# OATML-Markslab/ProteinGym

Hardware: AMD Instinct MI355X
Metric: mutants scored/sec (ESM-1v 650M masked-marginal) (higher is better)
Workload: dtype f16x3 (fp32 operands split into 2 fp16 planes, 3 fp16 MFMAs per product, fp32 accumulate)

## Files before the change

proteingym_amd/csrc/api_model.hip:

```cpp
#include "model.h"

namespace pgmi {

static thread_local char g_err[1024] = "";
void set_error(const char* fmt, ...) {
    va_list ap;
    va_start(ap, fmt);
    vsnprintf(g_err, sizeof(g_err), fmt, ap);
    va_end(ap);
}

int prof_drain(pgmi_model* m) {
    if (m->events_used == 0) return PGMI_OK;
    PGMI_HIP(hipStreamSynchronize(m->stream));
    for (size_t i = 0; i < m->events_used; ++i) {
        float ms = 0.f;
        PGMI_HIP(hipEventElapsedTime(&ms, m->events[i].start, m->events[i].stop));
        m->prof_ms[m->events[i].cls] += ms;
    }
    m->events_used = 0;
    return PGMI_OK;
}

int check_cfg(const pgmi_config* c) {
// ... 312 lines not shown
                         : cfg->arch == PGMI_ARCH_ESM3 ? esm3_weight_count(cfg, arch_arg)
                         : cfg->arch == PGMI_ARCH_ESMIF1 ? if1_weight_count(cfg, arch_arg) : pgmi_weight_count(cfg);
    if (need < 0) { set_error("causal decoder pos_kind %d: must be PGMI_GPT_POS_ROTARY or PGMI_GPT_POS_LEARNED", arch_arg); return PGMI_EINVAL; }
    if (!w || n_weights != need) {
        set_error("weight blob has %lld elements, config needs %lld", (long long)n_weights, (long long)need);
        return PGMI_EINVAL;
    }
    const int ndev = pgmi_device_count();
    if (ndev <= 0) { set_error("no HIP device visible (libpgmi has no CPU fallback)"); return PGMI_ENODEV; }
    if (device < 0 || device >= ndev) { set_error("device %d out of range (%d visible)", device, ndev); return PGMI_EINVAL; }
    PGMI_HIP(hipSetDevice(device));
    pgmi_model* m = new pgmi_model();
    m->cfg = *cfg;
    m->device = device;
    if (hipStreamCreateWithFlags(&m->stream, hipStreamNonBlocking) != hipSuccess) { set_error("hipStreamCreate failed"); delete m; return PGMI_EHIP; }
    m->dh = cfg->embed_dim / cfg->heads;
    m->rot_halves = m->dh > 2 * kHeadDim ? 4 : m->dh > kHeadDim ? 2 : 1;
    m->Hs = cfg->heads * m->rot_halves;
    m->Da = m->Hs * kHeadDim;
    m->ln_eps = cfg->ln_eps > 0.f ? cfg->ln_eps : 1e-5f;
    m->max_rows = std::max(cfg->max_rows > 0 ? cfg->max_rows : 98304, 2048);
    const size_t V = cfg->vocab;
    const std::vector<float> zeros(std::max({3 * (size_t)m->Da, (V + 63) / 64 * 64, (size_t)cfg->embed_dim, V, (size_t)cfg->heads}), 0.0f);
    rc = dev_upload(m->allocs, &m->zeros, zeros.data(), zeros.size());
    m->fc1_cols = cfg->ffn_dim;
    if (!rc) switch (cfg->arch) {
        case PGMI_ARCH_TRANCEPTION: rc = create_tranception(m, cfg, w, n_weights); break;
        case PGMI_ARCH_MSA: rc = create_msa(m, cfg, w, n_weights); break;
        case PGMI_ARCH_PROGEN2: rc = create_progen2(m, cfg, w, n_weights, arch_arg); break;
        case PGMI_ARCH_GPT: rc = create_gpt(m, cfg, w, n_weights, arch_arg); break;
        case PGMI_ARCH_ESMC: rc = create_esmc(m, cfg, w, n_weights); break;
        case PGMI_ARCH_SAPROT: rc = create_saprot(m, cfg, w, n_weights, arch_arg); break;
        case PGMI_ARCH_POET: rc = create_poet(m, cfg, w, n_weights, arch_arg); break;
        case PGMI_ARCH_PROGEN3: rc = create_progen3(m, cfg, w, n_weights, pg3); break;
        case PGMI_ARCH_ESM3: rc = create_esm3(m, cfg, w, n_weights, arch_arg); break;
        case PGMI_ARCH_ESMIF1: rc = create_esmif1(m, cfg, w, n_weights, arch_arg); break;
        default: rc = create_esm(m, cfg, w, n_weights);
    }
    if (!rc) rc = alloc_workspace(m);
    if (rc) { pgmi_model_destroy(m); return rc; }
    m->keep_rows = env_int("PGMI_KEEP_ROWS", 1);
    gemm_options_from_env();
    m->gemm_variant = env_int("PGMI_GEMM_VARIANT", 0);
    *out = m;
    return PGMI_OK;
}

}

extern "C" {

void pgmi_model_destroy(pgmi_model* m) {
    if (!m) return;
    hipSetDevice(m->device);
    if (m->stream) hipStreamSynchronize(m->stream);
    for (pgmi_assay* a : m->assays) {
        for (void* p : a->allocs) hipFree(p);
        a->allocs.clear();
        a->m = nullptr;
    }
    m->assays.clear();
    for (pgmi_pppl* q : m->pppls) {
        for (void* p : q->allocs) hipFree(p);
        q->allocs.clear();
        q->m = nullptr;
    }
    m->pppls.clear();
    for (auto& e : m->events) { hipEventDestroy(e.start); hipEventDestroy(e.stop); }
    if (m->moe.counts_host) hipHostFree(m->moe.counts_host);
    for (void* p : m->allocs) hipFree(p);
    if (m->stream) hipStreamDestroy(m->stream);
    delete m;
}

int pgmi_model_device(const pgmi_model* m) { return m ? m->device : -1; }

int pgmi_set_option(const char* name, int64_t value) {
    if (!name) { set_error("null option name"); return PGMI_EINVAL; }
    int rc = gemm_set_option(name, (long long)value);
    if (rc) rc = att_set_option(name, (long long)value);
    if (rc) rc = eve_set_option(name, (long long)value);
    if (rc) rc = mpnn_set_option(name, (long long)value);
    if (rc) rc = unirep_set_option(name, (long long)value);
    if (rc) set_error("unknown option '%s' (gemm_half_tail, gemm_max_rows, att_xcd_local, att_v3, eve_max_rows, eve_fixed_sample, eve_prior_batch, mpnn_max_rows, unirep_max_rows)", name);
    return rc;
}

int pgmi_synchronize(pgmi_model* m) {
    if (!m) { set_error("null model"); return PGMI_EINVAL; }
    PGMI_HIP(hipStreamSynchronize(m->stream));
    return PGMI_OK;
}

int pgmi_profile_enable(pgmi_model* m, int on) {
    if (!m) { set_error("null model"); return PGMI_EINVAL; }
    int rc = prof_drain(m);
    m->prof = on != 0;
    return rc;
}

int pgmi_profile_reset(pgmi_model* m) {
    if (!m) { set_error("null model"); return PGMI_EINVAL; }
    int rc = prof_drain(m);
    for (int i = 0; i < PGMI_K_COUNT; ++i) { m->prof_ms[i] = 0; m->prof_n[i] = 0; m->prof_flops[i] = 0; m->prof_bytes[i] = 0; }
    return rc;
}

int pgmi_profile_get(pgmi_model* m, int k, double* ms, int64_t* launches, double* flops, double* bytes) {
    if (!m || k < 0 || k >= PGMI_K_COUNT) { set_error("bad argument"); return PGMI_EINVAL; }
    int rc = prof_drain(m);
    if (rc) return rc;
    if (ms) *ms = m->prof_ms[k];
    if (launches) *launches = m->prof_n[k];
    if (flops) *flops = m->prof_flops[k];
    if (bytes) *bytes = m->prof_bytes[k];
    return PGMI_OK;
}

}
```

proteingym_amd/csrc/api_ops.hip:

```cpp
#include "model.h"

static inline float rebuild_split(unsigned short h, unsigned short l) {
    _Float16 a, b;
    memcpy(&a, &h, 2); memcpy(&b, &l, 2);
    return (float)a + (float)b * (1.0f / kLoScale);
}

extern "C" {

int pgmi_op_layernorm(int device, const float* x, const float* w, const float* b, int rows, int D, float eps, float* y) {
    if (!x || !w || !b || !y || rows <= 0 || D <= 0 || D % 4) { set_error("bad argument"); return PGMI_EINVAL; }
    if (pgmi_device_count() <= 0) { set_error("no HIP device visible"); return PGMI_ENODEV; }
    PGMI_HIP(hipSetDevice(device));
    std::vector<void*> pool;
    float *dx, *dw, *db, *dy;
    int rc = 0;
    if ((rc = dev_upload(pool, &dx, x, (size_t)rows * D)) || (rc = dev_upload(pool, &dw, w, (size_t)D)) ||
        (rc = dev_upload(pool, &db, b, (size_t)D)) || (rc = dev_alloc(pool, &dy, (size_t)rows * D))) {
        for (void* p : pool) hipFree(p);
        return rc;
    }
    launch_layernorm(dx, dw, db, rows, D, eps, dy, nullptr);
    hipError_t e = hipMemcpy(y, dy, (size_t)rows * D * 4, hipMemcpyDeviceToHost);
    for (void* p : pool) hipFree(p);
// ... 86 lines not shown
}

static GemmLaunch op_gemm(const unsigned short* a16, const W16& w16, const float* bias, int M, int N, int K, int variant) {
    GemmLaunch g;
    g.A = a16; g.W = w16.p; g.out_scale = w16.out_scale;
    g.bias = bias;
    g.M = M; g.N = N; g.K = K;
    g.variant = variant;
    return g;
}

int pgmi_op_gemm(int device, int precision, const float* A, const float* W, const float* bias, const float* residual,
                 int M, int N, int K, int epilogue, float* C) {
    if (!A || !W || !C || M <= 0 || N <= 0 || K <= 0) { set_error("bad argument"); return PGMI_EINVAL; }
    if (precision != PGMI_PREC_FP32 && precision != PGMI_PREC_F16X3 && precision != PGMI_PREC_BF16) { set_error("unknown precision %d", precision); return PGMI_EINVAL; }
    if (pgmi_device_count() <= 0) { set_error("no HIP device visible"); return PGMI_ENODEV; }
    PGMI_HIP(hipSetDevice(device));
    gemm_options_from_env();
    std::vector<void*> pool;
    float *dA, *dW = nullptr, *dB = nullptr, *dR = nullptr, *dC;
    int rc = 0;
    if ((rc = dev_upload(pool, &dA, A, (size_t)M * K)) ||
        (precision == PGMI_PREC_FP32 && (rc = dev_upload(pool, &dW, W, (size_t)N * K))) ||
        (bias && (rc = dev_upload(pool, &dB, bias, (size_t)N))) ||
        (residual && (rc = dev_upload(pool, &dR, residual, (size_t)M * N))) ||
        (rc = dev_alloc(pool, &dC, (size_t)M * N))) {
        for (void* p : pool) hipFree(p);
        return rc;
    }
    const int epi = epilogue & 255;
    const bool split_planes = (epilogue & 256) != 0;
    if (epi == EPI_SWIGLU && (!split_planes || precision != PGMI_PREC_F16X3 || (N % 64))) {
        for (void* p : pool) hipFree(p);
        set_error("SwiGLU GEMM op: precision f16x3 with the split-plane output (epilogue 4 + 256), N %% 64 == 0");
        return PGMI_EINVAL;
    }
    if (epi == EPI_RELU && precision != PGMI_PREC_F16X3) {
        for (void* p : pool) hipFree(p);
        set_error("ReLU GEMM op: precision f16x3 only");
        return PGMI_EINVAL;
    }
    if (split_planes && (precision == PGMI_PREC_FP32 || residual || (N % (precision == PGMI_PREC_F16X3 ? 32 : 4)))) {
        for (void* p : pool) hipFree(p);
        set_error("16-bit-plane GEMM op: f16x3 (N %% 32 == 0) or bf16 (N %% 4 == 0), no residual");
        return PGMI_EINVAL;
    }
    if (precision == PGMI_PREC_FP32) {
        rc = launch_gemm_f32(dA, dW, dB, dR, dC, M, N, K, epi, nullptr);
    } else {
        const bool bf = precision == PGMI_PREC_BF16;
        const int planes = bf ? 1 : 2;
        W16 w16;
        unsigned short* a16 = nullptr;
        rc = make_w16(pool, W, (size_t)N * K, (size_t)K, precision, nullptr, &w16);
        if (!rc) rc = dev_alloc(pool, &a16, (size_t)M * K * planes);
        if (!rc) {
            launch_split16(dA, (int64_t)M * K, 1.0f, bf ? 1 : 2, K, a16, nullptr);
            GemmLaunch g = op_gemm(a16, w16, dB, M, N, K, env_int("PGMI_GEMM_VARIANT", 0));
            g.epilogue = epi; g.bf = bf;
            if (split_planes) {
                unsigned short* c16 = nullptr;
                const int No = epi == EPI_SWIGLU ? N / 2 : N;
                rc = dev_alloc(pool, &c16, (size_t)M * N * 2);
                g.out16 = c16;
                if (!rc) rc = launch_gemm16(g);
                if (!rc) {
                    std::vector<unsigned short> h((size_t)M * N * 2);
                    hipError_t e2 = hipMemcpy(h.data(), c16, h.size() * 2, hipMemcpyDeviceToHost);
                    if (e2 != hipSuccess) { set_error("gemm op failed: %s", hipGetErrorString(e2)); rc = PGMI_EHIP; }
                    for (size_t m = 0; m < (size_t)M && !rc && bf; ++m)
                        for (int n = 0; n < N; ++n) {
                            const unsigned int u = (unsigned int)h[m * N + n] << 16;
                            memcpy(&C[m * N + n], &u, 4);
                        }
                    for (size_t m = 0; m < (size_t)M && !rc && !bf; ++m)
                        for (int n = 0; n < No; ++n) {
                            const size_t o = ki_off(m, n, No);
                            C[m * No + n] = rebuild_split(h[o], h[o + 32]);
                        }
                }
                for (void* p : pool) hipFree(p);
                return rc;
            }
            g.residual = dR; g.out32 = dC;
            rc = launch_gemm16(g);
        }
    }
    hipError_t e = hipMemcpy(C, dC, (size_t)M * N * 4, hipMemcpyDeviceToHost);
    for (void* p : pool) hipFree(p);
    if (rc) return rc;
    if (e != hipSuccess) { set_error("gemm op failed: %s", hipGetErrorString(e)); return PGMI_EHIP; }
    return PGMI_OK;
}

int pgmi_bench_gemm_ab(int device, int precision, int M, int N, int K, int epilogue, int split_out, const int* variants,
                       int n_variants, int rounds, int iters, double* ms_out) {
    if (M <= 0 || N <= 0 || K <= 0 || iters <= 0 || rounds <= 0 || n_variants <= 0 || !variants || !ms_out) { set_error("bad argument"); return PGMI_EINVAL; }
    if (pgmi_device_count() <= 0) { set_error("no HIP device visible"); return PGMI_ENODEV; }
    PGMI_HIP(hipSetDevice(device));
    gemm_options_from_env();
    std::vector<void*> pool;
    auto cleanup = [&]() { for (void* p : pool) hipFree(p); };
    std::vector<float> hA((size_t)M * K), hW((size_t)N * K), hb(N);
    unsigned int st = 12345u;
    auto rnd = [&]() { st = st * 1664525u + 1013904223u; return ((st >> 8) * (1.0f / 8388608.0f)) - 1.0f; };
    for (auto& v : hA) v = rnd();
    for (auto& v : hW) v = rnd() * 0.03f;
    for (auto& v : hb) v = rnd();
    float *dA, *dW = nullptr, *dB, *dC = nullptr;
    unsigned short *a16 = nullptr, *c16 = nullptr;
    int rc = 0;
    if ((rc = dev_upload(pool, &dA, hA.data(), hA.size())) || (rc = dev_upload(pool, &dB, hb.data(), hb.size()))) { cleanup(); return rc; }
    hipEvent_t e0, e1;
    PGMI_HIP(hipEventCreate(&e0));
    PGMI_HIP(hipEventCreate(&e1));
    const bool f32 = precision == PGMI_PREC_FP32;
    const bool bf = precision == PGMI_PREC_BF16;
    const int planes = bf ? 1 : 2;
    W16 w16;
    if (f32) {
        if ((rc = dev_upload(pool, &dW, hW.data(), hW.size())) || (rc = dev_alloc(pool, &dC, (size_t)M * N))) { cleanup(); return rc; }
    } else {
        if ((rc = make_w16(pool, hW.data(), hW.size(), (size_t)K, precision, nullptr, &w16)) ||
            (rc = dev_alloc(pool, &a16, (size_t)M * K * planes))) { cleanup(); return rc; }
        launch_split16(dA, (int64_t)M * K, 1.0f, bf ? 1 : 2, K, a16, nullptr);
        if (split_out == 1) rc = dev_alloc(pool, &c16, (size_t)M * N * planes);
        else if (split_out != 3) rc = dev_alloc(pool, &dC, (size_t)M * N);
        if (rc) { cleanup(); return rc; }
    }
    const bool fused_qkv = split_out == 3 && !f32 && !bf;
    const int Tq = (M % 288 == 0) ? 288 : M;
    unsigned short *qk16 = nullptr, *vt16 = nullptr;
    size_t qk_plane = 0, vt_plane = 0;
    if (fused_qkv) {
        if (N % 3 || (N / 3) % 64) { set_error("fused QKV bench needs N = 3 D, D %% 64 == 0"); cleanup(); return PGMI_EINVAL; }
        const size_t Tp = (size_t)(Tq + 31) / 32 * 32;
        qk_plane = (size_t)M * 2 * (N / 3);
        vt_plane = (size_t)(M / Tq) * (N / 3) * Tp;
        if ((rc = dev_alloc(pool, &qk16, qk_plane * 2)) || (rc = dev_alloc(pool, &vt16, vt_plane * 2))) { cleanup(); return rc; }
    }
    auto run = [&](int var) -> int {
        if (f32) return launch_gemm_f32(dA, dW, dB, split_out == 2 ? dC : nullptr, dC, M, N, K, epilogue, nullptr);
        GemmLaunch g = op_gemm(a16, w16, dB, M, N, K, var);
        if (fused_qkv) {
            g.out16 = qk16;
            g.qkv.vt16 = vt16; g.qkv.vt_plane = vt_plane; g.qkv.qk_plane = qk_plane;
            g.qkv.T = Tq; g.qkv.H = N / 3 / kHeadDim;
            return launch_gemm16(g);
        }
        g.epilogue = epilogue; g.bf = bf;
        if (split_out == 2) g.residual = dC;
        if (split_out == 1) g.out16 = c16; else g.out32 = dC;
        return launch_gemm16(g);
    };
    std::vector<std::vector<double>> samples(n_variants);
    for (int v = 0; v < n_variants && !rc; ++v) rc = run(variants[v] >= 0 ? variants[v] : env_int("PGMI_GEMM_VARIANT", 0));
    for (int r = 0; r < rounds && !rc; ++r)
        for (int v = 0; v < n_variants && !rc; ++v) {
            const int var = variants[v] >= 0 ? variants[v] : env_int("PGMI_GEMM_VARIANT", 0);
            hipEventRecord(e0, nullptr);
            for (int i = 0; i < iters && !rc; ++i) rc = run(var);
            hipEventRecord(e1, nullptr);
            hipError_t e = hipEventSynchronize(e1);
            float ms = 0.f;
            if (e == hipSuccess) e = hipEventElapsedTime(&ms, e0, e1);
            if (e != hipSuccess) { set_error("bench failed: %s", hipGetErrorString(e)); rc = PGMI_EHIP; }
            samples[v].push_back(ms / iters);
        }
// ... 620 lines not shown
```

proteingym_amd/csrc/gemm16x_kernel.h:

```cpp
#pragma once
#include <type_traits>

#include "common.h"

namespace pgmi {

typedef _Float16 h8 __attribute__((ext_vector_type(8)));
typedef _Float16 h4 __attribute__((ext_vector_type(4)));
typedef __bf16 b8 __attribute__((ext_vector_type(8)));
typedef unsigned int u32x4 __attribute__((ext_vector_type(4)));
typedef unsigned int u32x2 __attribute__((ext_vector_type(2)));

__device__ __forceinline__ f32x4 gelu_erf16(f32x4 x) {
    auto all = [](float v) { return f32x4{v, v, v, v}; };
    const f32x4 b = __builtin_elementwise_max(-__builtin_elementwise_abs(x), all(-6.0f));
    f32x4 q = __builtin_elementwise_fma(x, all(0.0f), all(3.309269596e-05f));
    q = __builtin_elementwise_fma(q, b, all(7.692188374e-04f));
    q = __builtin_elementwise_fma(q, b, all(8.080714382e-03f));
    q = __builtin_elementwise_fma(q, b, all(5.341210216e-02f));
    q = __builtin_elementwise_fma(q, b, all(-4.587709904e-01f));
    q = __builtin_elementwise_fma(q, b, all(1.151201725e+00f));
    q = __builtin_elementwise_fma(q, b, all(-9.999930859e-01f));
    const f32x4 e = {__builtin_amdgcn_exp2f(q[0]), __builtin_amdgcn_exp2f(q[1]), __builtin_amdgcn_exp2f(q[2]), __builtin_amdgcn_exp2f(q[3])};
    return __builtin_elementwise_fma(b, e, __builtin_elementwise_max(x, all(0.0f)));
}

__device__ __forceinline__ f32x4 gelu_tanh16(f32x4 x) {
    constexpr float c = -2.0f * 0.7978845608028654f * 1.4426950408889634f;
    f32x4 r;
#pragma unroll
    for (int e = 0; e < 4; ++e) {
        const float u = fmaf(0.044715f * x[e], x[e] * x[e], x[e]);
        r[e] = x[e] / (1.0f + __builtin_amdgcn_exp2f(c * u));
    }
    return r;
}

__device__ __forceinline__ f32x4 silu16(f32x4 x) {
    constexpr float c = -1.4426950408889634f;
    f32x4 r;
#pragma unroll
    for (int e = 0; e < 4; ++e) r[e] = x[e] / (1.0f + __builtin_amdgcn_exp2f(c * x[e]));
    return r;
}

struct QkvOut {
    unsigned short* vt16;
    size_t vt_plane;
    const float* cos_t;
    const float* sin_t;
    int T, H, Tp, rotary;
    int rot_halves;
};

template <bool BF>
__device__ __forceinline__ f32x16 mfma16(u32x4 a, u32x4 b, f32x16 c) {
    if constexpr (BF) {
        return __builtin_amdgcn_mfma_f32_32x32x16_bf16(__builtin_bit_cast(b8, a), __builtin_bit_cast(b8, b), c, 0, 0, 0);
    } else {
        return __builtin_amdgcn_mfma_f32_32x32x16_f16(__builtin_bit_cast(h8, a), __builtin_bit_cast(h8, b), c, 0, 0, 0);
    }
}

template <bool BF>
__device__ __forceinline__ f32x4 mfma16x16(u32x4 a, u32x4 b, f32x4 c) {
    if constexpr (BF) {
        return __builtin_amdgcn_mfma_f32_16x16x32_bf16(__builtin_bit_cast(b8, a), __builtin_bit_cast(b8, b), c, 0, 0, 0);
    } else {
        return __builtin_amdgcn_mfma_f32_16x16x32_f16(__builtin_bit_cast(h8, a), __builtin_bit_cast(h8, b), c, 0, 0, 0);
    }
}

template <typename T>
__device__ __forceinline__ void lds_put(unsigned char* p, T v) {
    *(__attribute__((address_space(3))) T*)(p) = v;
}

__device__ __forceinline__ unsigned short f32_to_bf16_rne(float f) {
    unsigned int u = __builtin_bit_cast(unsigned int, f);
    u += 0x7fffu + ((u >> 16) & 1u);
    return (unsigned short)(u >> 16);
}

struct TilePlan {
    int tiles_m, tiles_n;
    int n_main;
    int n_tail;
    int half;
    int group_m;
};

struct XMap {
    unsigned int a_row_bytes, w_row_bytes;
    unsigned int a_bytes, w_bytes;
    int k_run_log2;
    unsigned int a_run_bytes, w_run_bytes;
    int tiles_per_batch, batch_inner;
    unsigned int a_b0, a_b1, w_b0, w_b1;
    long long c_b0, c_b1;
    int ldc;
    int o_ld;
    int o_rows_per_n64;
    int o_col_per_batch;
};

constexpr int XBM = 256, XBN = 256, XNT = 512, XCPR = 8;
constexpr int X_OP_CH = XBM * XCPR;
constexpr int X_STAGE = 2 * X_OP_CH;
constexpr int X_PATCH_BYTES = 72 * 1024;
constexpr size_t X_LDS_BYTES = (size_t)(X_STAGE * 16 + X_PATCH_BYTES);

__device__ __forceinline__ void x_tile_coords(int wgid, int tiles_m, int tiles_n, int& tm, int& tn, int GROUP_M) {
    const int width = GROUP_M * tiles_n;
    const int group = wgid / width, first_m = group * GROUP_M;
    const int gsz = min(tiles_m - first_m, GROUP_M);
    tm = first_m + (wgid % width) % gsz;
    tn = (wgid % width) / gsz;
}

template <int EPI, int OUT, bool XM = false, bool BF = false>
__global__ __launch_bounds__(XNT, 2) void gemm16x_kernel(
    const unsigned short* __restrict__ A, const unsigned short* __restrict__ W, const float* __restrict__ bias,
    const float* residual, float* Cf, unsigned short* Ch, size_t c_plane, int M, int N, int K, float out_scale,
    TilePlan tp, QkvOut qo, XMap xm_arg) {
    static_assert(!(XM && BF), "the batched / strided form is f16x3 only");
    constexpr unsigned int EB = BF ? 2u : 4u;
    const XMap xm = XM ? xm_arg : XMap{};
    constexpr int WN = 4, TMX = 8, TN = 4, LD = 4;
    extern __shared__ __attribute__((aligned(16))) u32x4 lds[];
    const int tid = threadIdx.x, lane = tid & 63;
    const int wave = __builtin_amdgcn_readfirstlane(tid >> 6);
    const int wm = wave / WN, wn = wave % WN;
    const int r = lane & 15, kq = lane >> 4;
    const bool late = wave >= 4;
    unsigned char* const patches = reinterpret_cast<unsigned char*>(lds + X_STAGE);

    const int row_lo = tid >> 3, c8 = tid & 7, sw8 = (row_lo >> 1) & 7;
    const int csrc = c8 ^ sw8;
    const unsigned int a_row_bytes = xm.a_row_bytes ? xm.a_row_bytes : (unsigned int)K * EB;
    const unsigned int w_row_bytes = xm.w_row_bytes ? xm.w_row_bytes : (unsigned int)K * EB;
    const __amdgpu_buffer_rsrc_t rsA = __builtin_amdgcn_make_buffer_rsrc(const_cast<unsigned short*>(A), 0, (int)(xm.a_bytes ? xm.a_bytes : (unsigned int)M * (unsigned int)K * EB), 0x00020000);
    const __amdgpu_buffer_rsrc_t rsW = __builtin_amdgcn_make_buffer_rsrc(const_cast<unsigned short*>(W), 0, (int)(xm.w_bytes ? xm.w_bytes : (unsigned int)N * (unsigned int)K * EB), 0x00020000);
    unsigned int a_off[LD], w_off[LD];
    int m0 = 0, n0 = 0, a_ld = LD, batch = 0;
    unsigned int a_base = 0, w_base = 0;
    bool half_item = false;
    const int nk = BF ? K / 64 : K / 32;
    const int n_items = tp.n_main + tp.n_tail;
    auto decode = [&](int item) {
        const bool all_half = tp.half == 2;
        int wgid;
        if (item < tp.n_main || all_half) {
            const int nwg = all_half ? n_items : tp.n_main, xcd = item & 7, q = nwg >> 3, r8 = nwg & 7;
            wgid = (xcd < r8 ? xcd * (q + 1) : r8 * (q + 1) + (xcd - r8) * q) + (item >> 3);
        } else {
            wgid = tp.n_main + ((item - tp.n_main) >> 1);
        }
        batch = 0;
        if (xm.tiles_per_batch) {
            batch = wgid / xm.tiles_per_batch;
            wgid -= batch * xm.tiles_per_batch;
            const int bi = batch % xm.batch_inner, bo = batch / xm.batch_inner;
            a_base = __builtin_amdgcn_readfirstlane((unsigned int)bi * xm.a_b0 + (unsigned int)bo * xm.a_b1);
            w_base = __builtin_amdgcn_readfirstlane((unsigned int)bi * xm.w_b0 + (unsigned int)bo * xm.w_b1);
            batch = __builtin_amdgcn_readfirstlane(batch);
        }
        int tm, tn;
        x_tile_coords(wgid, tp.tiles_m, tp.tiles_n, tm, tn, tp.group_m);
        half_item = all_half || (tp.half && item >= tp.n_main);
        a_ld = half_item ? LD / 2 : LD;
        m0 = __builtin_amdgcn_readfirstlane(all_half ? tm * (XBM / 2) : tm * XBM + (half_item ? ((item - tp.n_main) & 1) * (XBM / 2) : 0));
        n0 = __builtin_amdgcn_readfirstlane(tn * XBN);
#pragma unroll
        for (int i = 0; i < LD; ++i) {
            a_off[i] = (unsigned int)min(m0 + row_lo + 64 * i, M - 1) * a_row_bytes + (unsigned int)csrc * 16u;
            w_off[i] = (unsigned int)min(n0 + row_lo + 64 * i, N - 1) * w_row_bytes + (unsigned int)csrc * 16u;
        }
    };
    auto issue_tile = [&](int kt, int buf) {
        u32x4* base = lds + buf * X_STAGE + wave * 64;
        const int run = kt >> xm.k_run_log2, in_run = kt - (run << xm.k_run_log2);
        const int ka = (int)(a_base + (xm.a_run_bytes ? (unsigned int)run * xm.a_run_bytes + (unsigned int)in_run * 128u : (unsigned int)kt * 128u));
        const int kw = (int)(w_base + (xm.w_run_bytes ? (unsigned int)run * xm.w_run_bytes + (unsigned int)in_run * 128u : (unsigned int)kt * 128u));
#pragma unroll
        for (int i = 0; i < LD; ++i)
            if (i < a_ld)
                __builtin_amdgcn_raw_ptr_buffer_load_lds(rsA, (__attribute__((address_space(3))) void*)(base + XNT * i), 16, (int)a_off[i], ka, 0, 0);
#pragma unroll
        for (int i = 0; i < LD; ++i)
            __builtin_amdgcn_raw_ptr_buffer_load_lds(rsW, (__attribute__((address_space(3))) void*)(base + X_OP_CH + XNT * i), 16, (int)w_off[i], kw, 0, 0);
    };
    auto phase = [&]() {
        __builtin_amdgcn_sched_barrier(0);
        __builtin_amdgcn_s_waitcnt(0xC07F);
        __builtin_amdgcn_s_barrier();
        __builtin_amdgcn_sched_barrier(0);
    };
    auto phase_vm = [&]() {
        __builtin_amdgcn_sched_barrier(0);
        __builtin_amdgcn_s_waitcnt(0x0070);
        __builtin_amdgcn_s_barrier();
        __builtin_amdgcn_sched_barrier(0);
    };

    f32x4 acc[TN][TMX];
    u32x4 af[2][TMX / 2], wf[2][TN], whs[TN];
    const int fsw = (r >> 1) & 7;
    auto read_frags = [&](auto tmc, auto hc, const u32x4* Ab, const u32x4* Wb) {
        constexpr int TM = decltype(tmc)::value, TH = TM / 2, H = decltype(hc)::value;
#pragma unroll
        for (int p = 0; p < 2; ++p) {
            const int c = (p * 4 + kq) ^ fsw;
#pragma unroll
            for (int i = 0; i < TH; ++i) af[p][i] = Ab[((wm * TM + H * TH + i) * 16 + r) * XCPR + c];
            if constexpr (H == 0)
#pragma unroll
                for (int j = 0; j < TN; ++j) wf[p][j] = Wb[((wn * TN + j) * 16 + r) * XCPR + c];
        }
    };
    auto scale_whi = [&]() {
        typedef _Float16 h2 __attribute__((ext_vector_type(2)));
        const h2 sc = {(_Float16)(1.0f / kLoScale), (_Float16)(1.0f / kLoScale)};
#pragma unroll
        for (int j = 0; j < TN; ++j)
#pragma unroll
            for (int e = 0; e < 4; ++e) {
                const unsigned int u = wf[0][j][e];
                const h2 t = __builtin_bit_cast(h2, u) * sc;
                whs[j][e] = __builtin_bit_cast(unsigned int, t);
            }
    };
    auto mfmas = [&](auto tmc, auto hc) {
        constexpr int TM = decltype(tmc)::value, TH = TM / 2, H = decltype(hc)::value;
        if constexpr (BF) {
#pragma unroll
            for (int p = 0; p < 2; ++p)
#pragma unroll
                for (int j = 0; j < TN; ++j)
#pragma unroll
                    for (int i = 0; i < TH; ++i) acc[j][H * TH + i] = mfma16x16<true>(wf[p][j], af[p][i], acc[j][H * TH + i]);
            return;
        }
        if constexpr (H == 0) scale_whi();
#pragma unroll
        for (int j = 0; j < TN; ++j)
#pragma unroll
            for (int i = 0; i < TH; ++i) acc[j][H * TH + i] = mfma16x16<false>(wf[1][j], af[0][i], acc[j][H * TH + i]);
#pragma unroll
        for (int j = 0; j < TN; ++j)
#pragma unroll
            for (int i = 0; i < TH; ++i) acc[j][H * TH + i] = mfma16x16<false>(whs[j], af[1][i], acc[j][H * TH + i]);
#pragma unroll
        for (int j = 0; j < TN; ++j)
#pragma unroll
            for (int i = 0; i < TH; ++i) acc[j][H * TH + i] = mfma16x16<false>(wf[0][j], af[0][i], acc[j][H * TH + i]);
        if constexpr (H == 0) {
#pragma unroll
            for (int k = 0; k < 4 * TN; ++k) {
                __builtin_amdgcn_sched_group_barrier(0x008, 1, 0);
                __builtin_amdgcn_sched_group_barrier(0x002, 1, 0);
            }
            __builtin_amdgcn_sched_group_barrier(0x008, 3 * TN * TH - 4 * TN, 0);
        }
    };
    using H0 = std::integral_constant<int, 0>;
    using H1 = std::integral_constant<int, 1>;

    int item = blockIdx.x;
    if (item >= n_items) return;
    decode(item);
    issue_tile(0, 0);
    auto run_item = [&](auto tmc) -> bool {
        constexpr int TM = decltype(tmc)::value;
        phase_vm();
#pragma unroll
        for (int j = 0; j < TN; ++j)
#pragma unroll
            for (int i = 0; i < TM; ++i)
#pragma unroll
                for (int v = 0; v < 4; ++v) acc[j][i][v] = 0.0f;
        int cur = 0;
        if (late) phase();
        for (int kt = 0; kt < nk; ++kt) {
            const u32x4* Ab = lds + cur * X_STAGE;
            const u32x4* Wb = Ab + X_OP_CH;
            __builtin_amdgcn_s_setprio(0);
            if (kt + 1 < nk) issue_tile(kt + 1, cur ^ 1);
            read_frags(tmc, H0{}, Ab, Wb);
            phase();
            __builtin_amdgcn_s_setprio(1);
            mfmas(tmc, H0{});
            phase();
            __builtin_amdgcn_s_setprio(0);
            read_frags(tmc, H1{}, Ab, Wb);
            if (late) phase_vm(); else phase();
            __builtin_amdgcn_s_setprio(1);
            mfmas(tmc, H1{});
            if (!late) phase_vm(); else phase();
            cur ^= 1;
        }
        __builtin_amdgcn_s_setprio(0);
        if (!late) phase();

        const int em0 = m0, en0 = n0, eb = batch;
        item += gridDim.x;
        const bool more = item < n_items;
        if (more) {
            decode(item);
            issue_tile(0, 0);
        }

        if constexpr (OUT == 2) {
            const int Dm = N / 3;
            const int nb = en0 + wn * 64;
            if (nb < N) {
            const int which = nb / Dm, hcol = nb - which * Dm, hh = hcol >> 6;
            constexpr int SPQ = 144;
            unsigned char* patch_q = patches + wave * (2 * 32 * SPQ);
            const bool staged_q = which < 2;
            f32x4 bq0[2], bq1[2];
#pragma unroll
            for (int g = 0; g < 2; ++g) {
                bq0[g] = *reinterpret_cast<const f32x4*>(bias + nb + 16 * g + 4 * kq);
                bq1[g] = *reinterpret_cast<const f32x4*>(bias + nb + 32 + 16 * g + 4 * kq);
            }
#pragma unroll
            for (int g = 0; g < 2; ++g) asm volatile("" :: "v"(bq0[g]), "v"(bq1[g]));
#pragma unroll
            for (int ib = 0; ib < TM / 2; ++ib) {
#pragma unroll
            for (int s = 0; s < 2; ++s) {
                const int i = 2 * ib + s, prow = 16 * s + r;
                const int m = em0 + (wm * TM + i) * 16 + r;
                const bool row_ok = m < M;
                if (!row_ok) continue;
                const int bb = m / qo.T, t = m - bb * qo.T;
                f32x4 rc[2], rs[2];
                if (which < 2 && qo.rotary) {
                    const int tr = (min(t, qo.T - 1) * qo.rot_halves + (hh % qo.rot_halves)) * 64;
#pragma unroll
                    for (int g = 0; g < 2; ++g) {
                        rc[g] = *reinterpret_cast<const f32x4*>(qo.cos_t + tr + 16 * g + 4 * kq);
                        rs[g] = *reinterpret_cast<const f32x4*>(qo.sin_t + tr + 16 * g + 4 * kq);
                    }
                }
#pragma unroll
                for (int g = 0; g < 2; ++g) {
                    const int d0 = 16 * g + 4 * kq;
                    const f32x4 b0 = bq0[g], b1 = bq1[g];
                    float x0[4], x1[4];
#pragma unroll
                    for (int e = 0; e < 4; ++e) {
                        x0[e] = fmaf(acc[g][i][e], out_scale, b0[e]);
                        x1[e] = fmaf(acc[g + 2][i][e], out_scale, b1[e]);
                    }
                    if (which == 0) {
#pragma unroll
                        for (int e = 0; e < 4; ++e) { x0[e] *= kQLog2e; x1[e] *= kQLog2e; }
                    }
                    if (which < 2) {
                        if (qo.rotary) {
                            const f32x4 c1 = rc[g], s1 = rs[g], c2 = rc[g], s2 = rs[g];
#pragma unroll
                            for (int e = 0; e < 4; ++e) {
                                const float y0 = fmaf(x0[e], c1[e], (-x1[e]) * s1[e]);
                                const float y1 = fmaf(x1[e], c2[e], x0[e] * s2[e]);
                                x0[e] = y0;
                                x1[e] = y1;
                            }
                        }
                        h4 hi0, lo0, hi1, lo1;
#pragma unroll
                        for (int e = 0; e < 4; ++e) {
                            _Float16 a, b2;
                            split_act(x0[e], a, b2); hi0[e] = a; lo0[e] = b2;
                            split_act(x1[e], a, b2); hi1[e] = a; lo1[e] = b2;
                        }
                        unsigned char* cell = patch_q + prow * SPQ + d0 * 2;
                        lds_put(cell, hi0);
                        lds_put(cell + 32 * SPQ, lo0);
                        lds_put(cell + 64, hi1);
                        lds_put(cell + 32 * SPQ + 64, lo1);
                    } else {
                        const int tk = t & 31;
                        const int pos = (t & ~31) + ((tk & 0x13) | ((tk & 4) << 1) | ((tk & 8) >> 1));
                        unsigned short* col = qo.vt16 + (((size_t)bb * qo.H + hh) * kHeadDim + d0) * qo.Tp + pos;
#pragma unroll
                        for (int e = 0; e < 4; ++e) {
                            _Float16 a0, l0, a1, l1;
                            split_act(x0[e], a0, l0);
                            split_act(x1[e], a1, l1);
                            unsigned short* c0 = col + (size_t)e * qo.Tp;
                            unsigned short* c1p = c0 + (size_t)32 * qo.Tp;
// ... 298 lines not shown
```

proteingym_amd/csrc/gemm_f16.hip:

```cpp
#include <stdlib.h>
#include <string.h>
#include <algorithm>
#include <mutex>

#include "common.h"
#include "gemm16x_kernel.h"

namespace pgmi {

constexpr int kMaxDevices = 64;
static int g_num_cus[kMaxDevices];
static std::mutex g_xdev_mu;

static int x_num_cus() {
    int dev = 0;
    if (hipGetDevice(&dev) != hipSuccess || dev < 0 || dev >= kMaxDevices) dev = 0;
    std::lock_guard<std::mutex> lk(g_xdev_mu);
    int& n = g_num_cus[dev];
    if (!n) {
        hipDeviceProp_t prop;
        if (hipGetDeviceProperties(&prop, dev) == hipSuccess) n = prop.multiProcessorCount;
        if (n <= 0) n = 256;
        n -= n % 8;
        if (n <= 0) n = 8;
    }
    return n;
}

constexpr int kGroupM = 4, kGroupMWide = 8, kWideTilesN = 16;
struct GemmOptions { int half_tail = 1; long long max_rows = 0; bool half_tail_set = false, max_rows_set = false; };
static GemmOptions g_opt;
void gemm_options_from_env() {
    const char* h = getenv("PGMI_GEMM_HALF_TAIL");
    const char* r = getenv("PGMI_GEMM_MAX_ROWS");
    if (!g_opt.half_tail_set) g_opt.half_tail = h ? atoi(h) : 1;
    if (!g_opt.max_rows_set) g_opt.max_rows = r ? atoll(r) : 0;
}
int gemm_set_option(const char* name, long long value) {
    if (!strcmp(name, "gemm_half_tail")) {
        g_opt.half_tail_set = value >= 0;
        if (value >= 0) g_opt.half_tail = (int)value; else gemm_options_from_env();
        return PGMI_OK;
    }
    if (!strcmp(name, "gemm_max_rows")) {
        g_opt.max_rows_set = value >= 0;
        if (value >= 0) g_opt.max_rows = value; else gemm_options_from_env();
        return PGMI_OK;
    }
    return PGMI_EINVAL;
}

static int gemm_group_m(int variant) { return variant >= 1000 ? (variant - 1000) & 15 : 0; }

enum { X_OUT_F32 = 0, X_OUT_16 = 1, X_OUT_QKV = 2 };
using GemmKernel = decltype(&gemm16x_kernel<EPI_NONE, X_OUT_F32>);
struct GemmInst { int epi, out; bool xm, bf; GemmKernel fn; };
template <int EPI, int OUT, bool XM = false, bool BF = false>
static GemmInst inst() { return {EPI, OUT, XM, BF, gemm16x_kernel<EPI, OUT, XM, BF>}; }
static const GemmInst kGemmInst[] = {
    inst<EPI_NONE, X_OUT_F32>(),                   inst<EPI_NONE, X_OUT_16>(),                   inst<EPI_NONE, X_OUT_QKV>(),
    inst<EPI_GELU, X_OUT_F32>(),                   inst<EPI_GELU, X_OUT_16>(),
    inst<EPI_SQRELU, X_OUT_F32>(),                 inst<EPI_SQRELU, X_OUT_16>(),
    inst<EPI_GELU_TANH, X_OUT_F32>(),              inst<EPI_GELU_TANH, X_OUT_16>(),
    inst<EPI_SWIGLU, X_OUT_16>(),
    inst<EPI_RELU, X_OUT_F32>(),                   inst<EPI_RELU, X_OUT_16>(),
    inst<EPI_NONE, X_OUT_F32, false, true>(),      inst<EPI_NONE, X_OUT_16, false, true>(),      inst<EPI_NONE, X_OUT_QKV, false, true>(),
    inst<EPI_GELU, X_OUT_F32, false, true>(),      inst<EPI_GELU, X_OUT_16, false, true>(),
    inst<EPI_SQRELU, X_OUT_F32, false, true>(),    inst<EPI_SQRELU, X_OUT_16, false, true>(),
    inst<EPI_GELU_TANH, X_OUT_F32, false, true>(), inst<EPI_GELU_TANH, X_OUT_16, false, true>(),
    inst<EPI_NONE, X_OUT_F32, true>(),             inst<EPI_NONE, X_OUT_16, true>(),
};

static int launch_x(const GemmLaunch& g, int out, bool xm, size_t c_plane, int G, int n_items, const TilePlan& tp, const QkvOut& qo,
                    const XMap& xmap) {
    const GemmInst* k = nullptr;
    for (const GemmInst& i : kGemmInst)
        if (i.epi == g.epilogue && i.out == out && i.xm == xm && i.bf == g.bf) { k = &i; break; }
    if (!k) {
        set_error("gemm16: no kernel for epilogue %d, output kind %d, xmap %d, bf16 %d", g.epilogue, out, (int)xm, (int)g.bf);
        return PGMI_EINVAL;
    }
    hipError_t e = hipFuncSetAttribute(reinterpret_cast<const void*>(k->fn), hipFuncAttributeMaxDynamicSharedMemorySize, (int)X_LDS_BYTES);
    if (e != hipSuccess) { set_error("hipFuncSetAttribute: %s", hipGetErrorString(e)); return PGMI_EHIP; }
    hipLaunchKernelGGL(k->fn, dim3(std::min(G, n_items)), dim3(XNT), X_LDS_BYTES, g.stream, g.A, g.W, g.bias, g.residual, g.out32, g.out16,
                       c_plane, g.M, g.N, g.K, g.out_scale, tp, qo, xmap);
    PGMI_HIP(hipGetLastError());
    return PGMI_OK;
}

static int launch_gemm16x_one(const GemmLaunch& g, int group_m) {
    const int M = g.M, N = g.N, K = g.K;
    const bool qkv = g.qkv.vt16 != nullptr;
    const unsigned long long eb = g.bf ? 2ull : 4ull;
    TilePlan tp{};
    tp.group_m = group_m > 0 ? group_m : ((N + XBN - 1) / XBN >= kWideTilesN ? kGroupMWide : kGroupM);
    tp.tiles_m = (M + XBM - 1) / XBM;
    tp.tiles_n = (N + XBN - 1) / XBN;
    const int T = tp.tiles_m * tp.tiles_n, G = x_num_cus();
    tp.n_main = T;
    if ((unsigned long long)std::max(M, N) * (unsigned long long)K * eb >= (1ull << 32) ||
        (g.out32 && (unsigned long long)M * (unsigned long long)N * 4ull >= (1ull << 31))) {
        set_error("gemm16x: operand of %d x %d split elements (or %d x %d outputs) exceeds the 32-bit offset range", std::max(M, N), K, M, N);
        return PGMI_EINVAL;
    }
    const int rem = T % G;
    if (g_opt.half_tail && !qkv && rem > 0 && 2 * rem <= G) {
        tp.n_main = T - rem; tp.half = 1; tp.n_tail = 2 * rem;
    }
    QkvOut qo{};
    if (qkv) qo = QkvOut{g.qkv.vt16, g.qkv.vt_plane, g.qkv.cos_t, g.qkv.sin_t, g.qkv.T, g.qkv.H, (g.qkv.T + 31) / 32 * 32, g.qkv.rotary, g.qkv.rot_halves};
    return launch_x(g, qkv ? X_OUT_QKV : g.out16 ? X_OUT_16 : X_OUT_F32, false, qkv ? g.qkv.qk_plane : 0, G, tp.n_main + tp.n_tail, tp, qo, XMap{});
}

int launch_gemm16_ex(const unsigned short* A, const unsigned short* W, float* Cf, unsigned short* Ch, int M, int N, int K,
                     float out_scale, XMap xm, int nbatch, hipStream_t s) {
    if (M <= 0 || N <= 0 || K <= 0 || (K % 64) != 0 || (N % 4) != 0 || (!Cf && !Ch) || (Cf && Ch) || nbatch < 1 ||
        (Ch && (N % 64) != 0) || (xm.a_run_bytes && (K / 32) % (1 << xm.k_run_log2) != 0)) {
        set_error("gemm16_ex: unsupported shape/args M=%d N=%d K=%d batches=%d", M, N, K, nbatch);
        return PGMI_EINVAL;
    }
    TilePlan tp{};
    tp.group_m = kGroupM;
    const int rows_last = M % XBM;
    const bool all_half = rows_last > 0 && rows_last <= XBM / 2;
    tp.tiles_m = all_half ? (M + XBM / 2 - 1) / (XBM / 2) : (M + XBM - 1) / XBM;
    tp.tiles_n = (N + XBN - 1) / XBN;
    const int per = tp.tiles_m * tp.tiles_n, T = per * nbatch, G = x_num_cus();
    xm.tiles_per_batch = per;
    if (xm.batch_inner < 1) xm.batch_inner = 1;
    if (all_half) { tp.half = 2; tp.n_main = 0; tp.n_tail = T; } else { tp.n_main = T; }
    GemmLaunch g;
    g.A = A; g.W = W; g.out_scale = out_scale;
    g.out32 = Cf; g.out16 = Ch;
    g.M = M; g.N = N; g.K = K;
    g.stream = s;
    return launch_x(g, Ch ? X_OUT_16 : X_OUT_F32, true, 0, G, T, tp, QkvOut{}, xm);
}

static int launch_gemm16x(const GemmLaunch& g) {
    const int M = g.M, N = g.N, K = g.K, group_m = gemm_group_m(g.variant);
    const bool qkv = g.qkv.vt16 != nullptr;
    const unsigned long long lim = (1ull << 32) - 1;
    const unsigned long long eb = g.bf ? 2ull : 4ull;
    if ((unsigned long long)N * (unsigned long long)K * eb > lim) {
        set_error("gemm16x: weight of %d x %d split elements exceeds the 32-bit offset range", N, K);
        return PGMI_EINVAL;
    }
    const long long test_rows = g_opt.max_rows;
    long long max_rows = (long long)(lim / ((unsigned long long)K * eb));
    if (g.out32) max_rows = std::min(max_rows, (long long)(((1ull << 31) - 1) / ((unsigned long long)N * 4ull)));
    if (test_rows > 0) max_rows = std::min(max_rows, test_rows);
    if (M <= max_rows) return launch_gemm16x_one(g, group_m);
    long long per = qkv ? (max_rows / g.qkv.T) * g.qkv.T : (max_rows / XBM) * XBM;
    if (per <= 0) per = qkv ? 0 : max_rows;
    if (per <= 0) { set_error("gemm16x: one sequence of %d tokens x K = %d exceeds the 32-bit offset range", g.qkv.T, K); return PGMI_EINVAL; }
    const size_t n_out16 = qkv ? (size_t)(2 * (N / 3)) : (size_t)(g.bf ? 1 : 2) * (g.epilogue == EPI_SWIGLU ? (size_t)N / 2 : (size_t)N);
    for (long long m0 = 0; m0 < M; m0 += per) {
        GemmLaunch c = g;
        c.M = (int)std::min<long long>(per, M - m0);
        c.A = g.A + (size_t)m0 * (size_t)K * (g.bf ? 1 : 2);
        if (g.residual) c.residual = g.residual + (size_t)m0 * N;
        if (g.out32) c.out32 = g.out32 + (size_t)m0 * N;
        if (g.out16) c.out16 = g.out16 + (size_t)m0 * n_out16;
        if (qkv) c.qkv.vt16 = g.qkv.vt16 + (size_t)(m0 / g.qkv.T) * (size_t)g.qkv.H * kHeadDim * (size_t)((g.qkv.T + 31) / 32 * 32);
        const int rc = launch_gemm16x_one(c, group_m);
        if (rc) return rc;
    }
    return PGMI_OK;
}

int launch_gemm16(const GemmLaunch& g) {
    const int M = g.M, N = g.N, K = g.K;
    const int k_step = g.bf ? 64 : 32;
    if (g.qkv.vt16) {
        const int D = N / 3, T = g.qkv.T;
        if (M <= 0 || K <= 0 || D <= 0 || N != 3 * D || (K % k_step) || (D % 64) || T <= 0 || M % T || g.qkv.rot_halves < 1 || !g.out16 || g.out32 ||
            g.residual || g.epilogue != EPI_NONE) {
            set_error("gemm16_qkv: unsupported shape M=%d D=%d K=%d T=%d", M, D, K, T);
            return PGMI_EINVAL;
        }
        return launch_gemm16x(g);
    }
    if (M <= 0 || N <= 0 || K <= 0 || (K % k_step) != 0 || (N % 4) != 0 || (!g.out32 && !g.out16) || (g.out32 && g.out16)) {
        set_error("gemm16: unsupported shape/args M=%d N=%d K=%d (K %% %d == 0, N %% 4 == 0 required)", M, N, K, k_step);
        return PGMI_EINVAL;
    }
    if (g.epilogue == EPI_SWIGLU && (g.bf || !g.out16 || g.residual || (N % 64) != 0)) {
        set_error("gemm16: the SwiGLU epilogue is f16x3 with split-plane output, no residual and N %% 64 == 0 (N = %d)", N);
        return PGMI_EINVAL;
    }
    if (!g.bf && g.out16 && (N % 32) != 0) {
        set_error("gemm16: split output needs N %% 32 == 0 (K-interleaved operand of the next GEMM), got %d", N);
        return PGMI_EINVAL;
    }
// ... 30 lines not shown
```

Baseline: 18530.

## Add phase-grouped persistent tile schedule with staggered half tiles in gemm16

Adds a phase-grouped work schedule to the persistent f16x3 GEMM kernel. Half of each XCD pair starts on a half-height tile, so tile completions are staggered across rounds, and the remainder is finished with a mix of full and half tiles, replacing the old half-tail-only split. The aim is less tail imbalance and fewer wave-quantization idle CUs. It also adds a gemm_cus option to cap the CU count, and the residual path in the test op now copies the residual into the output before launch. The new decode logic is more complex and assumes a grid that is a multiple of 8 with a 4-XCD-pair structure.

```diff
diff --git a/proteingym_amd/csrc/api_model.hip b/proteingym_amd/csrc/api_model.hip
--- a/proteingym_amd/csrc/api_model.hip
+++ b/proteingym_amd/csrc/api_model.hip
@@ -418,7 +418,7 @@
     if (rc) rc = eve_set_option(name, (long long)value);
     if (rc) rc = mpnn_set_option(name, (long long)value);
     if (rc) rc = unirep_set_option(name, (long long)value);
-    if (rc) set_error("unknown option '%s' (gemm_half_tail, gemm_max_rows, att_xcd_local, att_v3, eve_max_rows, eve_fixed_sample, eve_prior_batch, mpnn_max_rows, unirep_max_rows)", name);
+    if (rc) set_error("unknown option '%s' (gemm_half_tail, gemm_max_rows, gemm_phase_groups, gemm_cus, att_xcd_local, att_v3, eve_max_rows, eve_fixed_sample, eve_prior_batch, mpnn_max_rows, unirep_max_rows)", name);
     return rc;
 }
 
diff --git a/proteingym_amd/csrc/api_ops.hip b/proteingym_amd/csrc/api_ops.hip
--- a/proteingym_amd/csrc/api_ops.hip
+++ b/proteingym_amd/csrc/api_ops.hip
@@ -192,8 +192,12 @@
                 for (void* p : pool) hipFree(p);
                 return rc;
             }
-            g.residual = dR; g.out32 = dC;
-            rc = launch_gemm16(g);
+            if (dR && hipMemcpyAsync(dC, dR, (size_t)M * N * 4, hipMemcpyDeviceToDevice, nullptr) != hipSuccess) {
+                set_error("gemm op: copying the residual failed");
+                rc = PGMI_EHIP;
+            }
+            g.residual = dR ? dC : nullptr; g.out32 = dC;
+            if (!rc) rc = launch_gemm16(g);
         }
     }
     hipError_t e = hipMemcpy(C, dC, (size_t)M * N * 4, hipMemcpyDeviceToHost);
diff --git a/proteingym_amd/csrc/gemm16x_kernel.h b/proteingym_amd/csrc/gemm16x_kernel.h
--- a/proteingym_amd/csrc/gemm16x_kernel.h
+++ b/proteingym_amd/csrc/gemm16x_kernel.h
@@ -88,6 +88,7 @@
     int n_tail;
     int half;
     int group_m;
+    int phase, rounds, last_full;
 };
 
 struct XMap {
@@ -146,11 +147,40 @@
     unsigned int a_base = 0, w_base = 0;
     bool half_item = false;
     const int nk = BF ? K / 64 : K / 32;
-    const int n_items = tp.n_main + tp.n_tail;
-    auto decode = [&](int item) {
+    constexpr bool PG = !XM && OUT != 2;
+    const bool pg = PG && tp.phase != 0;
+    bool pg_b = false;
+    int pg_j = 0, pg_run = 0, pg_last = 0, pg_ts = 0, rnd = 0;
+    if (pg) {
+        const int xcd = blockIdx.x & 7, k = blockIdx.x >> 3, t = xcd >> 1, f = tp.last_full;
+        pg_b = xcd & 1;
+        pg_ts = gridDim.x >> 3;
+        pg_j = k * 4 + t;
+        pg_run = (pg_b ? 4 * tp.rounds + t * (tp.rounds - 1) : t * tp.rounds) * pg_ts + k;
+        pg_last = tp.n_main - f + t * (f >> 2) + min(t, f & 3) + k;
+    }
+    const int n_items = pg ? (tp.rounds + 1) * (int)gridDim.x : tp.n_main + tp.n_tail;
+    auto decode = [&](int item) -> bool {
         const bool all_half = tp.half == 2;
-        int wgid;
-        if (item < tp.n_main || all_half) {
+        int wgid, lower = (item - tp.n_main) & 1;
+        bool hf = tp.half && item >= tp.n_main;
+        if (pg) {
+            int hidx = pg_j;
+            bool last_full = false;
+            hf = rnd == 0 && pg_b;
+            if (rnd >= tp.rounds) {
+                if (pg_b && pg_j < tp.last_full) {
+                    last_full = true;
+                } else if (pg_b == (tp.last_full == 0) && pg_j < tp.n_tail) {
+                    hf = true;
+                    hidx = (int)(gridDim.x >> 1) + pg_j;
+                } else {
+                    return false;
+                }
+            }
+            wgid = hf ? tp.n_main + (hidx >> 1) : last_full ? pg_last : pg_run + (rnd - (pg_b ? 1 : 0)) * pg_ts;
+            lower = hidx & 1;
+        } else if (item < tp.n_main || all_half) {
             const int nwg = all_half ? n_items : tp.n_main, xcd = item & 7, q = nwg >> 3, r8 = nwg & 7;
             wgid = (xcd < r8 ? xcd * (q + 1) : r8 * (q + 1) + (xcd - r8) * q) + (item >> 3);
         } else {
@@ -167,15 +197,16 @@
         }
         int tm, tn;
         x_tile_coords(wgid, tp.tiles_m, tp.tiles_n, tm, tn, tp.group_m);
-        half_item = all_half || (tp.half && item >= tp.n_main);
+        half_item = all_half || hf;
         a_ld = half_item ? LD / 2 : LD;
-        m0 = __builtin_amdgcn_readfirstlane(all_half ? tm * (XBM / 2) : tm * XBM + (half_item ? ((item - tp.n_main) & 1) * (XBM / 2) : 0));
+        m0 = __builtin_amdgcn_readfirstlane(all_half ? tm * (XBM / 2) : tm * XBM + (half_item ? lower * (XBM / 2) : 0));
         n0 = __builtin_amdgcn_readfirstlane(tn * XBN);
 #pragma unroll
         for (int i = 0; i < LD; ++i) {
             a_off[i] = (unsigned int)min(m0 + row_lo + 64 * i, M - 1) * a_row_bytes + (unsigned int)csrc * 16u;
             w_off[i] = (unsigned int)min(n0 + row_lo + 64 * i, N - 1) * w_row_bytes + (unsigned int)csrc * 16u;
         }
+        return true;
     };
     auto issue_tile = [&](int kt, int buf) {
         u32x4* base = lds + buf * X_STAGE + wave * 64;
@@ -304,11 +335,9 @@
 
         const int em0 = m0, en0 = n0, eb = batch;
         item += gridDim.x;
-        const bool more = item < n_items;
-        if (more) {
-            decode(item);
-            issue_tile(0, 0);
-        }
+        ++rnd;
+        const bool more = item < n_items && decode(item);
+        if (more) issue_tile(0, 0);
 
         if constexpr (OUT == 2) {
             const int Dm = N / 3;
diff --git a/proteingym_amd/csrc/gemm_f16.hip b/proteingym_amd/csrc/gemm_f16.hip
--- a/proteingym_amd/csrc/gemm_f16.hip
+++ b/proteingym_amd/csrc/gemm_f16.hip
@@ -12,7 +12,7 @@
 static int g_num_cus[kMaxDevices];
 static std::mutex g_xdev_mu;
 
-static int x_num_cus() {
+static int x_num_cus_device() {
     int dev = 0;
     if (hipGetDevice(&dev) != hipSuccess || dev < 0 || dev >= kMaxDevices) dev = 0;
     std::lock_guard<std::mutex> lk(g_xdev_mu);
@@ -28,13 +28,22 @@
 }
 
 constexpr int kGroupM = 4, kGroupMWide = 8, kWideTilesN = 16;
-struct GemmOptions { int half_tail = 1; long long max_rows = 0; bool half_tail_set = false, max_rows_set = false; };
+constexpr int kPhaseGroupsDefault = 1;
+struct GemmOptions {
+    int half_tail = 1, phase_groups = kPhaseGroupsDefault, cus = 0;
+    long long max_rows = 0;
+    bool half_tail_set = false, max_rows_set = false, phase_groups_set = false, cus_set = false;
+};
 static GemmOptions g_opt;
 void gemm_options_from_env() {
     const char* h = getenv("PGMI_GEMM_HALF_TAIL");
     const char* r = getenv("PGMI_GEMM_MAX_ROWS");
+    const char* p = getenv("PGMI_GEMM_PHASE_GROUPS");
+    const char* c = getenv("PGMI_GEMM_CUS");
     if (!g_opt.half_tail_set) g_opt.half_tail = h ? atoi(h) : 1;
     if (!g_opt.max_rows_set) g_opt.max_rows = r ? atoll(r) : 0;
+    if (!g_opt.phase_groups_set) g_opt.phase_groups = p ? atoi(p) : kPhaseGroupsDefault;
+    if (!g_opt.cus_set) g_opt.cus = c ? atoi(c) : 0;
 }
 int gemm_set_option(const char* name, long long value) {
     if (!strcmp(name, "gemm_half_tail")) {
@@ -47,7 +56,23 @@
         if (value >= 0) g_opt.max_rows = value; else gemm_options_from_env();
         return PGMI_OK;
     }
+    if (!strcmp(name, "gemm_phase_groups")) {
+        g_opt.phase_groups_set = value >= 0;
+        if (value >= 0) g_opt.phase_groups = (int)value; else gemm_options_from_env();
+        return PGMI_OK;
+    }
+    if (!strcmp(name, "gemm_cus")) {
+        g_opt.cus_set = value >= 0;
+        if (value >= 0) g_opt.cus = (int)value; else gemm_options_from_env();
+        return PGMI_OK;
+    }
     return PGMI_EINVAL;
+}
+
+static int x_num_cus() {
+    const int n = x_num_cus_device();
+    if (g_opt.cus <= 0) return n;
+    return std::min(n, std::max(8, g_opt.cus - g_opt.cus % 8));
 }
 
 static int gemm_group_m(int variant) { return variant >= 1000 ? (variant - 1000) & 15 : 0; }
@@ -107,9 +132,20 @@
     if (g_opt.half_tail && !qkv && rem > 0 && 2 * rem <= G) {
         tp.n_main = T - rem; tp.half = 1; tp.n_tail = 2 * rem;
     }
+    int n_items = tp.n_main + tp.n_tail;
+    const int h = G / 2;
+    if (g_opt.phase_groups && g_opt.half_tail && !qkv && T >= 2 * G) {
+        const int R = (T + h / 2) / G, rest = T + h / 2 - R * G;
+        if (2 * rest <= 3 * h) {
+            const int f = 2 * rest <= h ? 0 : std::min(rest, h);
+            tp.phase = 1; tp.rounds = R; tp.last_full = f;
+            tp.n_main = h + (R - 1) * G + f; tp.half = 1; tp.n_tail = 2 * (rest - f);
+            n_items = (R + 1) * G;
+        }
+    }
     QkvOut qo{};
     if (qkv) qo = QkvOut{g.qkv.vt16, g.qkv.vt_plane, g.qkv.cos_t, g.qkv.sin_t, g.qkv.T, g.qkv.H, (g.qkv.T + 31) / 32 * 32, g.qkv.rotary, g.qkv.rot_halves};
-    return launch_x(g, qkv ? X_OUT_QKV : g.out16 ? X_OUT_16 : X_OUT_F32, false, qkv ? g.qkv.qk_plane : 0, G, tp.n_main + tp.n_tail, tp, qo, XMap{});
+    return launch_x(g, qkv ? X_OUT_QKV : g.out16 ? X_OUT_16 : X_OUT_F32, false, qkv ? g.qkv.qk_plane : 0, G, n_items, tp, qo, XMap{});
 }
 
 int launch_gemm16_ex(const unsigned short* A, const unsigned short* W, float* Cf, unsigned short* Ch, int M, int N, int K,
```

Result: no change. 18580 (median of 6 runs) (+0.3%).
